# Kolkir/mono_slam_framework

Hardware: AMD Instinct MI355X
Metric: frame-pairs/sec (extract+match) (higher is better)
Workload: dtype u8; 1 GPU; ORB extract+match, 1280x720 pairs, 1024 pairs/GPU/step resident in HBM, ratio 0.60; pairs_per_gpu=1024, width=1280, height=720, synth_mode=0, overflow_pairs=0, ranks=1, rccl_ranks=0

## Files before the change

mono_slam_framework_amd/csrc/orb_kernels.hip:

```cpp
#include <type_traits>
#include "orb_pipeline.h"

#include <math.h>
#include <stdlib.h>
#include <string.h>

#include "orb_pattern.h"

namespace msf {

constexpr int SW = TW + 2, SH = TH + 2;
constexpr int kTileCandCap = TW * TH / 4;
constexpr int kTileY0 = kEdge;

constexpr uint32_t kStatusOverflow = 1u;

__constant__ __attribute__((aligned(16))) signed char c_pattern[1024];
__constant__ uint32_t c_disc[2 * kDiscTasks];

__device__ __forceinline__ __amdgpu_buffer_rsrc_t uniform_rsrc(const void* p, uint32_t bytes) {
  const unsigned long long v = (unsigned long long)p;
  const uint32_t lo = (uint32_t)__builtin_amdgcn_readfirstlane((int)(uint32_t)v);
  const uint32_t hi = (uint32_t)__builtin_amdgcn_readfirstlane((int)(uint32_t)(v >> 32));
  return __builtin_amdgcn_make_buffer_rsrc((void*)(((unsigned long long)hi << 32) | lo), 0,
// ... 1401 lines not shown
                                                msf_keypoint* kp, uint32_t* kp_cnt, uint32_t* status) {
  __shared__ uint4 kept[kSelCap];
  constexpr int kRespCap = 4096;
  __shared__ __attribute__((aligned(16))) float resp[kRespCap];
  __shared__ __attribute__((aligned(16))) uint32_t keys[kSelCap];
  __shared__ uint32_t nkept;
  const int slot = slot0 + blockIdx.x, tid = threadIdx.x;
  msf_keypoint* out = kp + (long long)slot * kKpCap;
  uint32_t base = 0;
  bool overflow = false;
  for (int l = 0; l < g.nlevels; l++) {
    const OrbLevelInfo L = g.lv[l];
    const uint32_t n = s1_cnt[slot * kOrbLevels + l];
    const uint4* in = s1 + (long long)slot * g.s1_total + L.s1_off;
    const uint32_t keep = (uint32_t)L.quota;
    if (tid == 0) nkept = 0;
    const bool staged = n > keep && n <= (uint32_t)kRespCap;
    const uint32_t n4 = (n + 3) >> 2;
    if (staged)
      for (uint32_t i = tid; i < 4 * n4; i += 256) resp[i] = i < n ? __uint_as_float(in[i].y) : -INFINITY;
    __syncthreads();
    for (uint32_t i = tid; i < n; i += 256) {
      const uint4 e = in[i];
      bool k = true;
      if (n > keep) {
        const float v = __uint_as_float(e.y);
        uint32_t greater = 0;
        if (staged) {
          const float4* r4 = reinterpret_cast<const float4*>(resp);
          for (uint32_t j = 0; j < n4; j++) {
            const float4 r = r4[j];
            greater += (uint32_t)(r.x > v) + (uint32_t)(r.y > v) + (uint32_t)(r.z > v) + (uint32_t)(r.w > v);
          }
        } else {
          for (uint32_t j = 0; j < n; j++) greater += (__uint_as_float(in[j].y) > v) ? 1u : 0u;
        }
        k = greater < keep;
      }
      if (k) {
        const uint32_t q = atomicAdd(&nkept, 1u);
        if (q < (uint32_t)kSelCap) kept[q] = e;
      }
    }
    __syncthreads();
    uint32_t m = nkept;
    if (m > (uint32_t)kSelCap) { overflow = true; m = kSelCap; }
    if (base + m > (uint32_t)kKpCap) { overflow = true; m = kKpCap - base; }
    const uint32_t m4 = (m + 3) >> 2;
    for (uint32_t i = tid; i < 4 * m4; i += 256) keys[i] = i < m ? kept[i].x : 0xFFFFFFFFu;
    __syncthreads();
    for (uint32_t i = tid; i < m; i += 256) {
      const uint4 e = kept[i];
      uint32_t rank = 0;
      const uint4* k4 = reinterpret_cast<const uint4*>(keys);
      for (uint32_t j = 0; j < m4; j++) {
        const uint4 kk = k4[j];
        rank += (uint32_t)(kk.x < e.x) + (uint32_t)(kk.y < e.x) + (uint32_t)(kk.z < e.x) + (uint32_t)(kk.w < e.x);
      }
      msf_keypoint k;
      k.lx = e.x & 0xFFFF;
      k.ly = e.x >> 16;
      k.x = (float)k.lx * L.scale;
      k.y = (float)k.ly * L.scale;
      k.response = __uint_as_float(e.y);
      k.angle = -1.f;
      k.octave = l;
      k.fast_score = (int)e.z;
      out[base + rank] = k;
    }
    base += m;
    __syncthreads();
  }
  if (tid == 0) {
    kp_cnt[slot] = base;
    if (overflow) atomicOr(&status[slot], kStatusOverflow);
  }
}

__device__ __forceinline__ float fast_atan2_deg(float y, float x) {
  const float k = (float)(180.0 / 3.14159265358979323846);
  const float p1 = 0.9997878412794807f * k, p3 = -0.3258083974640975f * k, p5 = 0.1555786518463281f * k,
              p7 = -0.04432655554792128f * k;
  const float ax = fabsf(x), ay = fabsf(y);
  float a, c, c2;
  if (ax >= ay) {
    c = ay / (ax + (float)2.2204460492503131e-16);
    c2 = c * c;
    a = (((p7 * c2 + p5) * c2 + p3) * c2 + p1) * c;
  } else {
    c = ax / (ay + (float)2.2204460492503131e-16);
    c2 = c * c;
    a = 90.f - (((p7 * c2 + p5) * c2 + p3) * c2 + p1) * c;
  }
  if (x < 0) a = 180.f - a;
  if (y < 0) a = 360.f - a;
  return a;
}

__device__ __forceinline__ void det_sincosf(float t, float* s, float* c) {
  const double x = (double)t;
  const int k = (int)(x * 6.36619772367581382433e-01 + 0.5);
  const double kd = (double)k;
  const double r = (x - kd * 1.57079632673412561417e+00) - kd * 6.07710050650619224932e-11;
  const double z = r * r;
  double p = 1.58969099521155010221e-10;
  p = p * z + -2.50507602534068634195e-08;
  p = p * z + 2.75573137070700676789e-06;
  p = p * z + -1.98412698298579493134e-04;
  p = p * z + 8.33333333332248946124e-03;
  p = p * z + -1.66666666666666324348e-01;
  const double sr = r + (r * z) * p;
  double q = -1.13596475577881948265e-11;
  q = q * z + 2.08757232129817482790e-09;
  q = q * z + -2.75573143513906633035e-07;
  q = q * z + 2.48015872894767294178e-05;
  q = q * z + -1.38888888888741095749e-03;
  q = q * z + 4.16666666666666019037e-02;
  const double cr = (1.0 - 0.5 * z) + (z * z) * q;
  double sv, cv;
  switch (k & 3) {
    case 0: sv = sr; cv = cr; break;
    case 1: sv = cr; cv = -sr; break;
    case 2: sv = -sr; cv = -cr; break;
    default: sv = -cr; cv = sr; break;
  }
  *s = (float)sv;
  *c = (float)cv;
}

constexpr int PR = 22;
constexpr int PD = 2 * PR + 1;
constexpr int PP = 48;
constexpr int HP = 40;
constexpr int HC = 46;

template <bool HALF_UP, bool SUM256>
__global__ __launch_bounds__(256) void k_describe(OrbGeometry g, FrameSrc src, const uint8_t* pyr,
                                                  msf_keypoint* kp, const uint32_t* kp_cnt, uint8_t* desc) {
  __shared__ __attribute__((aligned(16))) uint8_t raw_s[4][PD * PP + 16];
  __shared__ __attribute__((aligned(16))) uint16_t hb_s[4][HP * HC];
  __shared__ uint32_t disc_s[2 * kDiscTasks];
  __shared__ __attribute__((aligned(16))) int pat_s[256];
  const int fi = blockIdx.y, slot = src.slot0 + fi;
  const int wave = __builtin_amdgcn_readfirstlane((int)(threadIdx.x >> 6)), lane = threadIdx.x & 63;
  for (int i = threadIdx.x; i < 2 * kDiscTasks; i += 256) disc_s[i] = c_disc[i];
  pat_s[threadIdx.x] = reinterpret_cast<const int*>(c_pattern)[threadIdx.x];
  __shared__ unsigned long long lvl_base_s[kOrbLevels];
  __shared__ int lvl_pitch_s[kOrbLevels];
  if (threadIdx.x < kOrbLevels) {
    int pt = 0;
    const uint8_t* bp = level_ptr(g, src, pyr, fi, threadIdx.x < g.nlevels ? (int)threadIdx.x : 0, &pt);
    lvl_base_s[threadIdx.x] = (unsigned long long)bp;
    lvl_pitch_s[threadIdx.x] = pt;
  }
  __syncthreads();
  const uint32_t count = min(kp_cnt[slot], (uint32_t)kKpCap);
  uint8_t* raw = raw_s[wave];
  uint16_t* hb = hb_s[wave];
  uint32_t* raw32 = reinterpret_cast<uint32_t*>(raw);
  constexpr int NPL = (PD * (PP / 4) + 63) / 64;
  const uint32_t kstride = gridDim.x * 4;
  uint32_t k = blockIdx.x * 4 + wave;
  uint32_t pre[NPL];
  int xo_pre = 0;
  auto meta = [&](uint32_t k_) -> uint3 {
    if (k_ >= count) return make_uint3(0u, 0u, 0u);
    const msf_keypoint* Kp = kp + (long long)slot * kKpCap + k_;
    return make_uint3((uint32_t)Kp->octave, (uint32_t)Kp->lx, (uint32_t)Kp->ly);
  };
  auto issue = [&](uint3 m) {
    const uint32_t lv = (uint32_t)__builtin_amdgcn_readfirstlane((int)m.x);
    const int mx = __builtin_amdgcn_readfirstlane((int)m.y), my = __builtin_amdgcn_readfirstlane((int)m.z);
    const uint32_t pitch_ = (uint32_t)__builtin_amdgcn_readfirstlane(lvl_pitch_s[lv]);
    const unsigned long long b64 = lvl_base_s[lv];
    const unsigned long long img_ = ((unsigned long long)(uint32_t)__builtin_amdgcn_readfirstlane((int)(b64 >> 32)) << 32) |
                                    (uint32_t)__builtin_amdgcn_readfirstlane((int)(uint32_t)b64);
    typedef const __attribute__((address_space(1))) uint8_t* gptr_t;
    const int ax = (mx - PR) & ~3;
    xo_pre = (mx - PR) - ax;
    gptr_t base = (gptr_t)(img_ + (unsigned long long)((long long)(my - PR) * (long long)pitch_ + ax));
    const uint32_t pm = pitch_ - (uint32_t)PP;
#pragma unroll
    for (int u = 0; u < NPL; u++) {
      const uint32_t i = (uint32_t)lane + 64u * (uint32_t)u;
      const uint32_t r = (i * 43691u) >> 19;
      const uint32_t off = mad_u24(r, pm, 4u * i);
      pre[u] = i < (uint32_t)(PD * (PP / 4)) ? *(const __attribute__((address_space(1))) uint32_t*)(base + off) : 0u;
    }
  };
  uint32_t* hb32 = reinterpret_cast<uint32_t*>(hb);
  const int blur_rl = (lane * 26) >> 8, blur_gq = lane - 10 * blur_rl;
  const int blur_rd = blur_rl * (2 * (PP / 4)) + blur_gq, blur_wr = blur_gq * (4 * (HC / 2)) + blur_rl;
  const bool blur_last = 18 + blur_rl < 23;
  const uint32_t samp_base = (uint32_t)(uintptr_t)(__attribute__((address_space(3))) uint16_t*)hb +
                             2u * (uint32_t)((PR - 3) * HC + (PR - 3)) - 2u * HC * 0x400000u - 2u * 0x4B400000u;
  uint3 m_cur = meta(k), m_next = meta(k + kstride);
  if (k < count) issue(m_cur);
  for (; k < count; k += kstride) {
    const bool active = true;
    msf_keypoint* K = kp + (long long)slot * kKpCap + k;
    const int l = (int)m_cur.x, cx = (int)m_cur.y, cy = (int)m_cur.z;
    (void)l; (void)cx; (void)cy;
    const int xo = xo_pre;
#pragma unroll
    for (int u = 0; u < NPL; u++) {
      const int i = lane + 64 * u;
      if (i < PD * (PP / 4)) raw32[i] = pre[u];
    }
    m_cur = m_next;
    if (k + kstride < count) issue(m_cur);
    m_next = meta(k + 2 * kstride);
    MSF_WAVE_SYNC();
    float angle = 0.f;
    if (active) {
      int m10 = 0, m01 = 0;
      {
        const int dw0 = 1 + ((xo + 2) >> 2);
        const uint32_t shf = (uint32_t)(xo + 2) & 3u;
#pragma unroll
        for (int it = 0; it < kDiscTasks / 64; it++) {
          const int t = it * 64 + lane;
          const int row = t >> 3, k = t & 7;
          const uint32_t* d = raw32 + (row + 7) * (PP / 4) + dw0 + k;
          const uint32_t pxw = __builtin_amdgcn_alignbyte(d[1], d[0], shf) ^ 0x80808080u;
          const uint32_t wu = disc_s[2 * t], wv = disc_s[2 * t + 1];
          m10 = __builtin_amdgcn_sdot4((int)pxw, (int)wu, m10, false);
          m01 = __builtin_amdgcn_sdot4((int)pxw, (int)wv, m01, false);
        }
      }
      m10 = (int)__builtin_amdgcn_readlane((int)wave_incl_scan((uint32_t)m10), 63);
      m01 = (int)__builtin_amdgcn_readlane((int)wave_incl_scan((uint32_t)m01), 63);
      angle = fast_atan2_deg((float)m01, (float)m10);
      {
        constexpr uint32_t T0 = 18, T1 = 34, T2 = SUM256 ? 48 : 49, T3 = SUM256 ? 56 : 55;
        constexpr uint32_t A0 = T0 | T1 << 8 | T2 << 16 | T3 << 24, B0 = T2 | T1 << 8 | T0 << 16;
        constexpr uint32_t A1 = T0 << 8 | T1 << 16 | T2 << 24, B1 = T3 | T2 << 8 | T1 << 16 | T0 << 24;
        constexpr uint32_t A2 = T0 << 16 | T1 << 24, B2 = T2 | T3 << 8 | T2 << 16 | T1 << 24, C2 = T0;
        constexpr uint32_t A3 = T0 << 24, B3 = T1 | T2 << 8 | T3 << 16 | T2 << 24, C3 = T1 | T0 << 8;
        auto row4 = [&](const uint32_t* d, uint32_t* o) {
          const uint32_t d0 = d[0], d1 = d[1], d2 = d[2], d3 = d[3];
          const uint32_t e0 = __builtin_amdgcn_alignbyte(d1, d0, xo), e1 = __builtin_amdgcn_alignbyte(d2, d1, xo);
          const uint32_t e2 = __builtin_amdgcn_alignbyte(d3, d2, xo);
          o[0] = __builtin_amdgcn_udot4(e0, A0, __builtin_amdgcn_udot4(e1, B0, 0u, false), false);
          o[1] = __builtin_amdgcn_udot4(e0, A1, __builtin_amdgcn_udot4(e1, B1, 0u, false), false);
          o[2] = __builtin_amdgcn_udot4(e0, A2, __builtin_amdgcn_udot4(e1, B2, __builtin_amdgcn_udot4(e2, C2, 0u, false), false), false);
          o[3] = __builtin_amdgcn_udot4(e0, A3, __builtin_amdgcn_udot4(e1, B3, __builtin_amdgcn_udot4(e2, C3, 0u, false), false), false);
        };
#pragma unroll
        for (int it = 0; it < 4; it++) {
          const uint32_t* d = raw32 + blur_rd + it * (12 * (PP / 4));
          uint32_t ou[4], ol[4];
          row4(d, ou);
          row4(d + PP / 4, ol);
          if (it < 3 || blur_last) {
            uint32_t* w = hb32 + blur_wr + it * 6;
#pragma unroll
            for (int j = 0; j < 4; j++) w[j * (HC / 2)] = ou[j] | (ol[j] << 16);
          }
        }
      }
    }
    MSF_WAVE_SYNC();
    if (active) {
      float a, b;
      float rad = angle;
      rad *= (float)(3.14159265358979323846 / 180.f);
      det_sincosf(rad, &b, &a);
      const int4 pk = *reinterpret_cast<const int4*>(&pat_s[lane * 4]);
      const int words[4] = {pk.x, pk.y, pk.z, pk.w};
      uint32_t nib = 0;
      constexpr uint32_t K2 = SUM256 ? 48 : 49, K3 = SUM256 ? 56 : 55;
      constexpr uint32_t P0 = 18u | 34u << 16, P1 = K2 | K3 << 16, P2 = K2 | 34u << 16, P3 = 18u;
#pragma unroll
      for (int t = 0; t < 4; t++) {
        uint32_t val[2];
#pragma unroll
        for (int e = 0; e < 2; e++) {
          const float px = (float)(signed char)(words[t] >> (16 * e));
          const float py = (float)(signed char)(words[t] >> (16 * e + 8));
          const uint32_t tx = __float_as_uint((px * a - py * b) + 12582912.f);
          const uint32_t ty = __float_as_uint((px * b + py * a) + 12582912.f);
          const uint32_t addr = mad_u24(tx, 2u * HC, (ty << 1) + samp_base);
          const __attribute__((address_space(3))) uint32_t* q =
              (const __attribute__((address_space(3))) uint32_t*)(uintptr_t)(addr & ~3u);
          const uint32_t sh = addr & 2u;
          const uint32_t d0 = q[0], d1 = q[1], d2 = q[2], d3 = q[3];
          const uint32_t w0 = __builtin_amdgcn_alignbyte(d1, d0, sh), w1 = __builtin_amdgcn_alignbyte(d2, d1, sh);
          const uint32_t w2 = __builtin_amdgcn_alignbyte(d3, d2, sh), w3 = __builtin_amdgcn_alignbyte(0u, d3, sh);
          const uint32_t sum = udot2_u16(w0, P0, udot2_u16(w1, P1, udot2_u16(w2, P2, udot2_u16(w3, P3, 0u))));
          const uint32_t r = HALF_UP ? (sum + 32768u) >> 16 : (sum + 0x7FFFu + ((sum >> 16) & 1u)) >> 16;
          val[e] = min(r, 255u);
        }
        nib |= (uint32_t)(val[0] < val[1]) << t;
      }
      const uint32_t hi = __shfl_down(nib, 1);
      if ((lane & 1) == 0) desc[((long long)slot * kKpCap + k) * 32 + (lane >> 1)] = (uint8_t)(nib | (hi << 4));
      if (lane == 0) K->angle = angle;
    }
    MSF_WAVE_SYNC();
  }
}

constexpr int kTrainChunk = 1024;
__global__ __launch_bounds__(256) void k_match(int n_pairs, const int32_t* slot_a, const int32_t* slot_b,
                                               const msf_keypoint* kp, const uint32_t* kp_cnt, const uint8_t* desc,
                                               const uint32_t* status, float ratio, msf_match* out, int cap,
                                               int32_t* n_out, int chunk, int slot_base, int max_slots) {
  __shared__ __attribute__((aligned(16))) unsigned long long train[kTrainChunk * 4];
  __shared__ uint32_t wave_cnt[4];
  __shared__ uint32_t running;
  const int pair = blockIdx.x, tid = threadIdx.x, lane = tid & 63, wave = tid >> 6;
  const int sa = slot_a ? slot_a[pair] : slot_base + pair;
  const int sb = slot_b ? slot_b[pair] : slot_base + n_pairs + pair;
  if (sa < 0 || sa >= max_slots || sb < 0 || sb >= max_slots || ((status[sa] | status[sb]) & kStatusOverflow)) {
    if (tid == 0) n_out[pair] = -1;
    return;
  }
  const uint32_t n1 = min(kp_cnt[sa], (uint32_t)kKpCap), n2 = min(kp_cnt[sb], (uint32_t)kKpCap);
  const unsigned long long* tsrc = reinterpret_cast<const unsigned long long*>(desc + (long long)sb * kKpCap * 32);
  if (tid == 0) running = 0;
  __syncthreads();
  const msf_keypoint* ka = kp + (long long)sa * kKpCap;
  const msf_keypoint* kb = kp + (long long)sb * kKpCap;
  msf_match* o = out + (long long)pair * cap;
  for (uint32_t q0 = 0; q0 < n1; q0 += 256) {
    const uint32_t q = q0 + tid;
    const bool have_q = q < n1;
    unsigned long long q0w = 0, q1w = 0, q2w = 0, q3w = 0;
    if (have_q) {
      const unsigned long long* qd =
          reinterpret_cast<const unsigned long long*>(desc + ((long long)sa * kKpCap + q) * 32);
      q0w = qd[0]; q1w = qd[1]; q2w = qd[2]; q3w = qd[3];
    }
    int d0 = 0x7fffffff, d1 = 0x7fffffff, i0 = -1;
    for (uint32_t t0 = 0; t0 < n2; t0 += chunk) {
      const uint32_t tn = min(n2 - t0, (uint32_t)chunk);
      __syncthreads();
      for (uint32_t i = tid; i < tn * 4; i += 256) train[i] = tsrc[(size_t)t0 * 4 + i];
      __syncthreads();
      if (have_q) {
        for (uint32_t t = 0; t < tn; t++) {
          const unsigned long long* tr = &train[t * 4];
          const int d = __popcll(q0w ^ tr[0]) + __popcll(q1w ^ tr[1]) + __popcll(q2w ^ tr[2]) + __popcll(q3w ^ tr[3]);
          if (d < d1) {
            if (d < d0) { d1 = d0; d0 = d; i0 = (int)(t0 + t); }
            else d1 = d;
          }
        }
      }
    }
    const bool pass = have_q && n2 >= 2 && ((float)d0 < ratio * (float)d1);
    const unsigned long long bal = __ballot(pass);
    const uint32_t before = __popcll(bal & ((1ull << lane) - 1ull));
    if (lane == 0) wave_cnt[wave] = __popcll(bal);
    __syncthreads();
    uint32_t off = running;
    for (int w = 0; w < wave; w++) off += wave_cnt[w];
    if (pass) {
      const uint32_t idx = off + before;
      if (idx < (uint32_t)cap) {
        msf_match m;
        m.x1 = (int)ka[q].x; m.y1 = (int)ka[q].y;
        m.x2 = (int)kb[i0].x; m.y2 = (int)kb[i0].y;
        o[idx] = m;
      }
    }
    __syncthreads();
    if (tid == 0) running += wave_cnt[0] + wave_cnt[1] + wave_cnt[2] + wave_cnt[3];
    __syncthreads();
  }
  if (tid == 0) n_out[pair] = (int32_t)running;
}

constexpr int kSplitBlocks = kKpCap / 64;
constexpr int kSplitMaxPairs = 128;
__global__ __launch_bounds__(256) void k_match_split(int n_pairs, const int32_t* slot_a, const int32_t* slot_b,
                                                     const msf_keypoint* kp, const uint32_t* kp_cnt,
                                                     const uint8_t* desc, const uint32_t* status, float ratio,
                                                     msf_match* out, int cap, int32_t* n_out, int chunk,
                                                     uint32_t* qres, uint32_t* done, int slot_base, int max_slots) {
  __shared__ __attribute__((aligned(16))) unsigned long long train[kTrainChunk * 4];
  __shared__ int part[3][4][64];
  __shared__ uint32_t wave_cnt[4];
  __shared__ uint32_t running, last_s;
  const int pair = blockIdx.y, qb = blockIdx.x, tid = threadIdx.x, lane = tid & 63, wave = tid >> 6;
  const int sa = slot_a ? slot_a[pair] : slot_base + pair;
  const int sb = slot_b ? slot_b[pair] : slot_base + n_pairs + pair;
  if (sa < 0 || sa >= max_slots || sb < 0 || sb >= max_slots || ((status[sa] | status[sb]) & kStatusOverflow)) {
    if (qb == 0 && tid == 0) n_out[pair] = -1;
    return;
  }
  const uint32_t n1 = min(kp_cnt[sa], (uint32_t)kKpCap), n2 = min(kp_cnt[sb], (uint32_t)kKpCap);
  const unsigned long long* tsrc = reinterpret_cast<const unsigned long long*>(desc + (long long)sb * kKpCap * 32);
  uint32_t* qr = qres + (long long)pair * kKpCap;
  const uint32_t q = (uint32_t)qb * 64u + lane;
  if ((uint32_t)qb * 64u < n1) {
    const bool have_q = q < n1;
    unsigned long long q0w = 0, q1w = 0, q2w = 0, q3w = 0;
    if (have_q) {
      const unsigned long long* qd = reinterpret_cast<const unsigned long long*>(desc + ((long long)sa * kKpCap + q) * 32);
      q0w = qd[0]; q1w = qd[1]; q2w = qd[2]; q3w = qd[3];
    }
    int d0 = 0x7fffffff, d1 = 0x7fffffff, i0 = 0x7fffffff;
    for (uint32_t t0 = 0; t0 < n2; t0 += chunk) {
      const uint32_t tn = min(n2 - t0, (uint32_t)chunk);
      __syncthreads();
      for (uint32_t i = tid; i < tn * 4; i += 256) train[i] = tsrc[(size_t)t0 * 4 + i];
      __syncthreads();
      const uint32_t ta = (tn * wave) >> 2, tb = (tn * (wave + 1)) >> 2;
      for (uint32_t t = ta; t < tb; t++) {
        const unsigned long long* tr = &train[t * 4];
        const int d = __popcll(q0w ^ tr[0]) + __popcll(q1w ^ tr[1]) + __popcll(q2w ^ tr[2]) + __popcll(q3w ^ tr[3]);
        if (d < d1) {
          if (d < d0) { d1 = d0; d0 = d; i0 = (int)(t0 + t); }
          else d1 = d;
        }
      }
    }
    part[0][wave][lane] = d0;
    part[1][wave][lane] = i0;
    part[2][wave][lane] = d1;
    __syncthreads();
    if (wave == 0) {
      int b0 = 0x7fffffff, bi = 0x7fffffff, b1 = 0x7fffffff;
#pragma unroll
      for (int w = 0; w < 4; w++) {
        const int e0 = part[0][w][lane], ei = part[1][w][lane], e1 = part[2][w][lane];
        if (e0 < b0 || (e0 == b0 && ei < bi)) { b1 = min(b0, e1); b0 = e0; bi = ei; }
        else b1 = min(b1, e0);
        b1 = min(b1, e1);
      }
      const bool pass = have_q && n2 >= 2 && ((float)b0 < ratio * (float)b1);
      if (have_q) qr[q] = pass ? (0x80000000u | (uint32_t)bi) : 0u;
    }
  }
  __threadfence();
  __syncthreads();
  if (tid == 0) last_s = atomicAdd(&done[pair], 1u) == (uint32_t)gridDim.x - 1u;
  __syncthreads();
  if (!last_s) return;
  __threadfence();
  if (tid == 0) { running = 0; done[pair] = 0; }
  __syncthreads();
  const msf_keypoint* ka = kp + (long long)sa * kKpCap;
  const msf_keypoint* kb = kp + (long long)sb * kKpCap;
  msf_match* o = out + (long long)pair * cap;
  for (uint32_t q0 = 0; q0 < n1; q0 += 256) {
    const uint32_t qq = q0 + tid;
    const uint32_t r = qq < n1 ? __hip_atomic_load(&qr[qq], __ATOMIC_RELAXED, __HIP_MEMORY_SCOPE_AGENT) : 0u;
    const bool pass = (r & 0x80000000u) != 0u;
    const unsigned long long bal = __ballot(pass);
    const uint32_t before = __popcll(bal & ((1ull << lane) - 1ull));
    if (lane == 0) wave_cnt[wave] = __popcll(bal);
    __syncthreads();
    uint32_t off = running;
    for (int w = 0; w < wave; w++) off += wave_cnt[w];
    if (pass) {
      const uint32_t idx = off + before;
      if (idx < (uint32_t)cap) {
        const uint32_t t = r & 0x7fffffffu;
        msf_match m;
        m.x1 = (int)ka[qq].x; m.y1 = (int)ka[qq].y;
        m.x2 = (int)kb[t].x; m.y2 = (int)kb[t].y;
        o[idx] = m;
      }
    }
    __syncthreads();
    if (tid == 0) running += wave_cnt[0] + wave_cnt[1] + wave_cnt[2] + wave_cnt[3];
    __syncthreads();
  }
  if (tid == 0) n_out[pair] = (int32_t)running;
}

OrbPipeline::~OrbPipeline() { destroy(); }

void OrbPipeline::destroy() {
  if (h_walk_abort_) hipHostFree(h_walk_abort_);
  h_walk_abort_ = nullptr;
  for (auto& set : evr_)
    for (auto& e : set.ev) {
      if (e) hipEventDestroy(e);
      e = nullptr;
    }
  ev_ok_ = false;
}

#define MSF_HIP_TRY(expr)                                                                 \
  do {                                                                                    \
    hipError_t e_ = (expr);                                                               \
    if (e_ != hipSuccess) return std::string(#expr) + ": " + hipGetErrorString(e_);       \
  } while (0)

void OrbPipeline::read_env() {
  if (const char* e = getenv("MSF_ORB_FAST_TAU")) {
    const int v = atoi(e) & ~1;
    if (v >= kFastT && v <= 254) force_tau_ = v;
  }
  if (const char* e = getenv("MSF_ORB_RESIZE_GENERIC")) resize_generic_ = atoi(e) != 0;
  if (const char* e = getenv("MSF_ORB_FAST_ONE_PART")) fast_two_part_ = atoi(e) == 0;
  if (const char* e = getenv("MSF_ORB_UNFUSED")) fused_ = atoi(e) == 0;
  if (getenv("MSF_TEST_HOOKS"))
    if (const char* e = getenv("MSF_ORB_TEST_STALL_FRAME")) test_stall_frame_ = atoi(e);
  if (const char* e = getenv("MSF_ORB_WALK_PER_LEVEL")) walk_per_level_ = atoi(e) != 0;
  if (const char* e = getenv("MSF_ORB_TAU_PREDICT")) {
    const int v = atoi(e);
    if (v >= 0 && v <= 2000) tau_predict_pct_ = v;
  }
  tau2_margin_pct_ = kTau2MarginPct;
  if (const char* e = getenv("MSF_ORB_TAU2_MARGIN_PCT")) {
    const int v = atoi(e);
    if (v >= 1 && v <= 10000) tau2_margin_pct_ = v;
  }
}

std::string OrbPipeline::init(const OrbOptions& o) {
  max_slots_ = o.max_slots;
  half_up_ = o.blur_half_up;
  blur_sum256_ = o.blur_sum256;
  profile_ = o.profile;
  force_tau_ = o.dense_fast ? kFastT : 0;
  stream_min_frames_ = o.stream_min_frames;
  read_env();

  OrbPlanRequest rq;
  rq.width = o.width;
  rq.height = o.height;
  rq.max_slots = o.max_slots;
  rq.work_frames = o.work_frames;
  rq.level_size_mul_inv = o.level_size_mul_inv;
  rq.resize_generic = resize_generic_;
  rq.force_tau = force_tau_;
  rq.stream_min_frames = stream_min_frames_;
  OrbPlan plan;
  const std::string err = plan_orb(rq, &plan);
  if (!err.empty()) return err;
  g_ = plan.g;
  prim_ = plan.prim;
  harris_ = plan.harris;
  work_frames_ = plan.work_frames;
  for (int l = 0; l < kOrbLevels; l++) resize_shared_[l] = plan.resize_shared[l];

  const OrbGeometry& g = g_;
  const size_t S = (size_t)max_slots_, Wk = (size_t)work_frames_;
  const size_t total = (size_t)(g.pool_base + (long long)g.pool_entries);
  MSF_HIP_TRY(d_pyr_.reserve(Wk * g.pyr_bytes));
  MSF_HIP_TRY(d_tab_.reserve(plan.tab.size() * sizeof(uint32_t)));
  MSF_HIP_TRY(hipMemcpy(d_tab_, plan.tab.data(), plan.tab.size() * sizeof(uint32_t), hipMemcpyHostToDevice));
  MSF_HIP_TRY(d_cand_cnt_.reserve(Wk * kOrbLevels * sizeof(uint32_t)));
  MSF_HIP_TRY(d_tau_.reserve(2 * Wk * kOrbLevels * sizeof(uint32_t)));
  MSF_HIP_TRY(hipMemset(d_tau_, 0, 2 * Wk * kOrbLevels * sizeof(uint32_t)));
  MSF_HIP_TRY(d_redo_.reserve((1 + Wk * kOrbLevels) * sizeof(uint32_t)));
  MSF_HIP_TRY(d_redo_hist_.reserve(Wk * kOrbLevels * 256 * sizeof(uint32_t)));
  MSF_HIP_TRY(hipMemset(d_redo_hist_, 0, Wk * kOrbLevels * 256 * sizeof(uint32_t)));
  MSF_HIP_TRY(d_redo_thr_.reserve(Wk * kOrbLevels * sizeof(uint32_t)));
  MSF_HIP_TRY(d_qstat_.reserve(Wk * kOrbLevels * kQStat * sizeof(uint32_t)));
  MSF_HIP_TRY(hipMemset(d_qstat_, 0, Wk * kOrbLevels * kQStat * sizeof(uint32_t)));
  MSF_HIP_TRY(d_cand_.reserve(total * sizeof(uint32_t)));
  MSF_HIP_TRY(d_cand_sc_.reserve(total));
  MSF_HIP_TRY(d_cmap_.reserve(Wk * kOrbLevels * sizeof(uint2)));
  MSF_HIP_TRY(hipMemset(d_cmap_, 0, Wk * kOrbLevels * sizeof(uint2)));
  MSF_HIP_TRY(d_walk_abort_.reserve(16));
  MSF_HIP_TRY(hipMemset(d_walk_abort_, 0, 16));
  MSF_HIP_TRY(hipHostMalloc(&h_walk_abort_, 16, hipHostMallocDefault));
  h_walk_abort_[0] = h_walk_abort_[1] = 0u;
  MSF_HIP_TRY(d_s1_cnt_.reserve(Wk * kOrbLevels * sizeof(uint32_t)));
  MSF_HIP_TRY(d_s1_.reserve(Wk * g.s1_total * sizeof(uint4)));
  MSF_HIP_TRY(d_kp_.reserve(S * kKpCap * sizeof(msf_keypoint)));
  MSF_HIP_TRY(d_desc_.reserve(S * kKpCap * 32));
  MSF_HIP_TRY(d_kp_cnt_.reserve(S * sizeof(uint32_t)));
  MSF_HIP_TRY(d_status_.reserve(S * sizeof(uint32_t)));
  MSF_HIP_TRY(d_qres_.reserve((size_t)kSplitMaxPairs * kKpCap * sizeof(uint32_t)));
  MSF_HIP_TRY(d_done_.reserve((size_t)kSplitMaxPairs * sizeof(uint32_t)));
  MSF_HIP_TRY(hipMemset(d_done_, 0, (size_t)kSplitMaxPairs * sizeof(uint32_t)));
  MSF_HIP_TRY(hipMemset(d_kp_cnt_, 0, S * sizeof(uint32_t)));
  MSF_HIP_TRY(hipMemset(d_status_, 0, S * sizeof(uint32_t)));
  MSF_HIP_TRY(hipMemset(d_cand_cnt_, 0, Wk * kOrbLevels * sizeof(uint32_t)));
  MSF_HIP_TRY(hipMemset(d_s1_cnt_, 0, Wk * kOrbLevels * sizeof(uint32_t)));
  MSF_HIP_TRY(hipMemcpyToSymbol(HIP_SYMBOL(c_pattern), k_orb_bit_pattern_31, 1024));
  MSF_HIP_TRY(hipMemcpyToSymbol(HIP_SYMBOL(c_disc), plan.disc.data(), sizeof(uint32_t) * 2 * kDiscTasks));
  if (profile_) {
    for (auto& set : evr_)
      for (auto& e : set.ev) MSF_HIP_TRY(hipEventCreate(&e));
    ev_ok_ = true;
  }
  return "";
}

__global__ __launch_bounds__(256) void k_fill_u32(uint32_t* a, uint32_t* b, uint32_t v, int n) {
  const int i = blockIdx.x * 256 + threadIdx.x;
  if (i < n) { a[i] = v; b[i] = v; }
}

hipError_t OrbPipeline::extract(const FrameSrc& src, int n, hipStream_t st) {
  if (n <= 0) return hipSuccess;
  if (src.slot0 < 0 || src.slot0 + n > max_slots_ || n > work_frames_) return hipErrorInvalidValue;
  last_src_ = src;
  last_n_ = n;
  if (h_walk_abort_ && !walk_per_level_ && __atomic_load_n(&h_walk_abort_[1], __ATOMIC_RELAXED) != 0u) {
    walk_per_level_ = true;
    degraded_note_ = true;
  }
  if (test_stall_frame_ >= 0 && test_stall_calls_++ > 0) test_stall_frame_ = -1;
  if (ev_ok_) ev_begin_call();
  const hipError_t e = extract_range(src, n, st, ev_ok_ ? ev_ : nullptr);
  if (ev_ok_) ev_extract_pending_ = true;
  return e;
}

hipError_t OrbPipeline::extract_range(const FrameSrc& src, int n, hipStream_t st, hipEvent_t* evs) {
  const OrbGeometry& g = g_;
  hipError_t e;
  const ptrdiff_t back = (ptrdiff_t)src.slot0;
  uint8_t* const d_pyr_ = this->d_pyr_ - back * g.pyr_bytes;
  uint32_t* const d_cand_cnt_ = this->d_cand_cnt_ - back * kOrbLevels;
  uint2* const d_cmap_ = this->d_cmap_ - back * kOrbLevels;
  uint32_t* const d_qstat_ = this->d_qstat_ - back * kOrbLevels * kQStat;
  uint32_t* const d_s1_cnt_ = this->d_s1_cnt_ - back * kOrbLevels;
  uint4* const d_s1_ = this->d_s1_ - back * g.s1_total;
  uint32_t* const d_redo_hist_ = this->d_redo_hist_ - back * kOrbLevels * 256;
  uint32_t* const d_redo_thr_ = this->d_redo_thr_ - back * kOrbLevels;
  if ((e = hipMemsetAsync(this->d_cand_cnt_, 0, (size_t)n * kOrbLevels * 4, st))) return e;
  if ((e = hipMemsetAsync(d_status_ + src.slot0, 0, (size_t)n * 4, st))) return e;
  if ((e = hipMemsetAsync(d_redo_, 0, 4, st))) return e;
  if (evs) hipEventRecord(evs[0], st);
  uint32_t* tau = d_tau_ - back * kOrbLevels;
  uint32_t* tau_first = d_tau_ + (ptrdiff_t)work_frames_ * kOrbLevels - back * kOrbLevels;
  const int force_tau = (force_tau_ == 0 && n < stream_min_frames_) ? kFastT : force_tau_;
  const bool dense = force_tau == kFastT;
  if (dense && (long long)n * g.cand_total > (long long)g.pool_entries) return hipErrorInvalidValue;
  hipLaunchKernelGGL(k_cand_reset, dim3((n * kOrbLevels + 255) / 256), dim3(256), 0, st, g, prim_, this->d_cmap_, n, dense ? 1 : 0);
  const int dyn = (fast_two_part_ && force_tau == 0) ? 1 : 0;
  bool fused = fused_ && !dense && g.total_tiles > 0;
  for (int l = 1; l < g.nlevels; l++) fused = fused && g.lv[l].wk_fused != 0;
  auto launch_resize = [&](int l) {
    const OrbLevelInfo& L = g.lv[l];
    const int sw16 = (g.lv[l - 1].w + 16 + 15) & ~15;
    const int groups = (L.w + 3) >> 2;
    int rth = 8;
    const int threads = 256;
    while (rth > 4 && ((rth * 5 + 3) / 4 + 3) * sw16 > 60000) rth -= 4;
    const int lds_rows = (rth * 5 + 3) / 4 + 3;
    const uint32_t magic_n16 = (uint32_t)(0x100000000ull / (uint32_t)(sw16 >> 4)) + 1u;
    const uint32_t magic_groups = groups > 1 ? (uint32_t)(0x100000000ull / (uint32_t)groups) + 1u : 0u;
    hipLaunchKernelGGL(resize_shared_[l] ? k_resize<true> : k_resize<false>, dim3((L.h + rth - 1) / rth, n), dim3(threads),
                       (size_t)lds_rows * sw16 + 8 * kResizeMaxRows, st, g, src, d_pyr_, d_tab_, l, rth, lds_rows, magic_n16,
                       magic_groups);
  };
  auto launch_walk = [&](int l_lo, int l_hi, int chain, int resize_mask, int predict_pct) {
    long long per_frame = 0;
    for (int l = l_lo; l <= l_hi; l++) per_frame += 1 + g.lv[l].wk_nx * g.lv[l].wk_ny;
    const long long wgs = 8ll * ((n + 7) / 8) * per_frame;
    hipLaunchKernelGGL(k_walk, dim3((unsigned)wgs), dim3(64), 0, st, g, src, d_pyr_, d_tab_, tau, tau_first, d_qstat_,
                       d_cand_cnt_, d_cand_, d_cand_sc_, d_cmap_, d_redo_, d_redo_ + 1, d_status_, d_walk_abort_, l_lo, l_hi, n,
// ... 304 lines not shown
```

Measured before the change: 162,500 frame-pairs/sec.

## Compute Hamming distances in k_match with int8 MFMA bit-expanded dot products

```diff
diff --git a/mono_slam_framework_amd/csrc/orb_kernels.hip b/mono_slam_framework_amd/csrc/orb_kernels.hip
--- a/mono_slam_framework_amd/csrc/orb_kernels.hip
+++ b/mono_slam_framework_amd/csrc/orb_kernels.hip
@@ -1727,11 +1727,31 @@
 }
 
 constexpr int kTrainChunk = 1024;
+
+constexpr int kMatchS = kKpCap;
+constexpr int kMatchPadKey = 1 << 30;
+static_assert(kMatchS == 2048, "k_match reads the train index from the low 11 bits of a key");
+typedef int match_v4i __attribute__((ext_vector_type(4)));
+
+template <int BIT>
+__device__ __forceinline__ void match_expand(unsigned long long w, match_v4i (&f)[4]) {
+  const uint32_t half[2] = {(uint32_t)w, (uint32_t)(w >> 32)};
+#pragma unroll
+  for (int e = 0; e < 16; e++) {
+    const uint32_t h = half[e >> 3];
+    const int k = e & 7;
+    f[e >> 2][e & 3] = (int)((k <= BIT ? h << (BIT - k) : h >> (k - BIT)) & (0x01010101u << BIT));
+  }
+}
+
+__device__ __forceinline__ int match_med3(int a, int b, int c) { return max(min(a, b), min(max(a, b), c)); }
+
 __global__ __launch_bounds__(256) void k_match(int n_pairs, const int32_t* slot_a, const int32_t* slot_b,
                                                const msf_keypoint* kp, const uint32_t* kp_cnt, const uint8_t* desc,
                                                const uint32_t* status, float ratio, msf_match* out, int cap,
                                                int32_t* n_out, int chunk, int slot_base, int max_slots) {
   __shared__ __attribute__((aligned(16))) unsigned long long train[kTrainChunk * 4];
+  __shared__ __attribute__((aligned(16))) int32_t seed[kTrainChunk];
   __shared__ uint32_t wave_cnt[4];
   __shared__ uint32_t running;
   const int pair = blockIdx.x, tid = threadIdx.x, lane = tid & 63, wave = tid >> 6;
@@ -1748,32 +1768,68 @@
   const msf_keypoint* ka = kp + (long long)sa * kKpCap;
   const msf_keypoint* kb = kp + (long long)sb * kKpCap;
   msf_match* o = out + (long long)pair * cap;
+  const int col = lane & 15, grp = lane >> 4;
   for (uint32_t q0 = 0; q0 < n1; q0 += 256) {
     const uint32_t q = q0 + tid;
     const bool have_q = q < n1;
-    unsigned long long q0w = 0, q1w = 0, q2w = 0, q3w = 0;
-    if (have_q) {
+    const bool wave_q = q0 + (uint32_t)wave * 64u < n1;
+    match_v4i qf[4][4];
+    int pop_q = 0;
+    if (wave_q) {
       const unsigned long long* qd =
-          reinterpret_cast<const unsigned long long*>(desc + ((long long)sa * kKpCap + q) * 32);
-      q0w = qd[0]; q1w = qd[1]; q2w = qd[2]; q3w = qd[3];
-    }
-    int d0 = 0x7fffffff, d1 = 0x7fffffff, i0 = -1;
+          reinterpret_cast<const unsigned long long*>(desc + ((long long)sa * kKpCap + q0 + wave * 64) * 32);
+#pragma unroll
+      for (int j = 0; j < 4; j++) match_expand<5>(qd[(16 * j + col) * 4 + grp], qf[j]);
+      pop_q = __popcll(qd[lane * 4]) + __popcll(qd[lane * 4 + 1]) + __popcll(qd[lane * 4 + 2]) + __popcll(qd[lane * 4 + 3]);
+    }
+    int best[4], second[4];
+#pragma unroll
+    for (int j = 0; j < 4; j++) best[j] = second[j] = 0x7fffffff;
     for (uint32_t t0 = 0; t0 < n2; t0 += chunk) {
       const uint32_t tn = min(n2 - t0, (uint32_t)chunk);
+      const uint32_t ntile = (tn + 15u) >> 4;
       __syncthreads();
       for (uint32_t i = tid; i < tn * 4; i += 256) train[i] = tsrc[(size_t)t0 * 4 + i];
       __syncthreads();
-      if (have_q) {
-        for (uint32_t t = 0; t < tn; t++) {
-          const unsigned long long* tr = &train[t * 4];
-          const int d = __popcll(q0w ^ tr[0]) + __popcll(q1w ^ tr[1]) + __popcll(q2w ^ tr[2]) + __popcll(q3w ^ tr[3]);
-          if (d < d1) {
-            if (d < d0) { d1 = d0; d0 = d; i0 = (int)(t0 + t); }
-            else d1 = d;
-          }
+      for (uint32_t r = tid; r < ntile * 16; r += 256) {
+        const unsigned long long* tr = &train[r * 4];
+        seed[r] = r < tn ? kMatchS * (__popcll(tr[0]) + __popcll(tr[1]) + __popcll(tr[2]) + __popcll(tr[3])) + (int)(t0 + r)
+                         : kMatchPadKey;
+      }
+      __syncthreads();
+      if (wave_q) {
+        for (uint32_t tile = 0; tile < ntile; tile++) {
+          match_v4i tf[4];
+          match_expand<7>(train[(tile * 16 + col) * 4 + grp], tf);
+          const match_v4i sd = *reinterpret_cast<const match_v4i*>(&seed[tile * 16 + grp * 4]);
+          match_v4i acc[4] = {sd, sd, sd, sd};
+#pragma unroll
+          for (int s = 0; s < 4; s++)
+#pragma unroll
+            for (int j = 0; j < 4; j++) acc[j] = __builtin_amdgcn_mfma_i32_16x16x64_i8(tf[s], qf[j][s], acc[j], 0, 0, 0);
+#pragma unroll
+          for (int j = 0; j < 4; j++)
+#pragma unroll
+            for (int r = 0; r < 4; r++) {
+              second[j] = match_med3(best[j], second[j], acc[j][r]);
+              best[j] = min(best[j], acc[j][r]);
+            }
         }
       }
     }
+    int kb0 = 0x7fffffff, kb1 = 0x7fffffff;
+#pragma unroll
+    for (int j = 0; j < 4; j++) {
+      int b = best[j], s = second[j];
+#pragma unroll
+      for (int x = 16; x <= 32; x <<= 1) {
+        const int b2 = __shfl_xor(b, x), s2 = __shfl_xor(s, x);
+        s = min(max(b, b2), min(s, s2));
+        b = min(b, b2);
+      }
+      if (grp == j) { kb0 = b; kb1 = s; }
+    }
+    const int d0 = (kb0 >> 11) + pop_q, d1 = (kb1 >> 11) + pop_q, i0 = kb0 & (kMatchS - 1);
     const bool pass = have_q && n2 >= 2 && ((float)d0 < ratio * (float)d1);
     const unsigned long long bal = __ballot(pass);
     const uint32_t before = __popcll(bal & ((1ull << lane) - 1ull));
```

Result: no change. 162,200 frame-pairs/sec, median of 3 (-0.2%).
